# gwenzhang/GGA

Hardware: AMD Instinct MI355X
Metric: kitti_frames_per_sec_gga_train_step (higher is better)
Workload: dtype f32 tensors; products on 2 x f16 operand planes (block-scaled), f32 accumulate - measured no less accurate than fp32 kernels: per convolution 0.7 x (dense) / 0.7-1.2 x (sparse) the RMS error of an fp32 FMA chain vs float64, whole-step losses over 8 seeds <= 2.5e-5 from float64 (fp32 CPU step: <= 1.6

## Files before the change

### gga_amd/csrc/pfn.hip

```cpp
#include "gga_common.h"

__device__ __forceinline__ int64_t pfn_valid_rows(int64_t m, const int32_t* __restrict__ num_valid) {
    if (!num_valid) return m;
    const int64_t v = *num_valid;
    return v < m ? (v < 0 ? 0 : v) : m;
}

#define PFN_C 64
#define PFN_F 10
#define PFN_NM 65
#define PFN_SAVED 238

struct PfnGeom {
    float vx, vy, vz, xo, yo, zo;
};

__device__ __forceinline__ void pfn_decorate(const float4 p, const float mean[3], const float cen[3], float f[PFN_F]) {
    f[0] = p.x - cen[0]; f[1] = p.y - cen[1]; f[2] = p.z - cen[2]; f[3] = p.w;
    f[4] = p.x - mean[0]; f[5] = p.y - mean[1]; f[6] = p.z - mean[2];
    f[7] = f[0]; f[8] = f[1]; f[9] = f[2];
}

__device__ __forceinline__ void pfn_pillar_consts(const float4* __restrict__ pts, int n, const int4 co,
                                                  const PfnGeom g, float mean[3], float cen[3]) {
    float sx = 0.f, sy = 0.f, sz = 0.f;
    for (int p = 0; p < n; ++p) { const float4 q = pts[p]; sx += q.x; sy += q.y; sz += q.z; }
    const float fn = (float)n;
    mean[0] = sx / fn; mean[1] = sy / fn; mean[2] = sz / fn;
    float tx = (float)co.w * g.vx, ty = (float)co.z * g.vy, tz = (float)co.y * g.vz;
    asm volatile("" : "+v"(tx), "+v"(ty), "+v"(tz));
    cen[0] = tx + g.xo; cen[1] = ty + g.yo; cen[2] = tz + g.zo;
}

__global__ __launch_bounds__(256) void pfn_moments_kernel(const float4* __restrict__ voxels,
                                                         const int32_t* __restrict__ num_points,
                                                         const int4* __restrict__ coors, int64_t m,
                                                         const int32_t* __restrict__ num_valid, int P,
                                                         PfnGeom g, double* __restrict__ partials) {
    m = pfn_valid_rows(m, num_valid);
    double acc[PFN_NM];
#pragma unroll
    for (int i = 0; i < PFN_NM; ++i) acc[i] = 0.0;
    for (int64_t v = (int64_t)blockIdx.x * 256 + threadIdx.x; v < m; v += (int64_t)gridDim.x * 256) {
        int n = num_points[v];
        n = n < P ? n : P;
        if (n <= 0) continue;
        const float4* pts = voxels + v * P;
        float mean[3], cen[3];
        pfn_pillar_consts(pts, n, coors[v], g, mean, cen);
        float loc[PFN_NM];
#pragma unroll
        for (int i = 0; i < PFN_NM; ++i) loc[i] = 0.f;
        for (int p = 0; p < n; ++p) {
            float f[PFN_F];
            pfn_decorate(pts[p], mean, cen, f);
            int k = PFN_F;
#pragma unroll
            for (int a = 0; a < PFN_F; ++a) {
                loc[a] += f[a];
#pragma unroll
                for (int b = a; b < PFN_F; ++b) loc[k++] += f[a] * f[b];
            }
        }
#pragma unroll
        for (int i = 0; i < PFN_NM; ++i) acc[i] += (double)loc[i];
    }
    __shared__ double sh[4][PFN_NM];
#pragma unroll
    for (int i = 0; i < PFN_NM; ++i) {
        const double s = wave_sum(acc[i]);
        if ((threadIdx.x & 63) == 0) sh[threadIdx.x >> 6][i] = s;
    }
    __syncthreads();
    if (threadIdx.x < PFN_NM)
        partials[(int64_t)blockIdx.x * PFN_NM + threadIdx.x] =
            (sh[0][threadIdx.x] + sh[1][threadIdx.x]) + (sh[2][threadIdx.x] + sh[3][threadIdx.x]);
}

__global__ __launch_bounds__(64) void pfn_stats_kernel(const double* __restrict__ partials, int nblocks,
                                                      int64_t m, const int32_t* __restrict__ num_valid, int P,
                                                      const float* __restrict__ weight,
                                                      const float* __restrict__ gamma, const float* __restrict__ beta,
                                                      float eps, float momentum, int training,
                                                      float* __restrict__ running_mean, float* __restrict__ running_var,
                                                      double* __restrict__ saved, float* __restrict__ scale_shift) {
    __shared__ double S[PFN_NM];
    const int c = threadIdx.x;
    double rows = (double)pfn_valid_rows(m, num_valid) * (double)P;
    rows = rows > 0.0 ? rows : 1.0;
    if (c == 0) saved[PFN_SAVED] = rows;
    if (training) {
        for (int i = c; i < PFN_NM; i += 64) {
            double s = 0.0;
#pragma unroll 16
            for (int b = 0; b < nblocks; ++b) s += partials[(int64_t)b * PFN_NM + i];
            S[i] = s;
        }
        __syncthreads();
        double S1[PFN_F], S2[PFN_F][PFN_F];
        int k = PFN_F;
        for (int a = 0; a < PFN_F; ++a) {
            S1[a] = S[a];
            for (int b = a; b < PFN_F; ++b) { S2[a][b] = S[k]; S2[b][a] = S[k]; ++k; }
        }
        double w[PFN_F];
        for (int a = 0; a < PFN_F; ++a) w[a] = (double)weight[c * PFN_F + a];
        double m1 = 0.0, m2 = 0.0;
        for (int a = 0; a < PFN_F; ++a) {
            m1 += w[a] * S1[a];
            double t = 0.0;
            for (int b = 0; b < PFN_F; ++b) t += S2[a][b] * w[b];
            m2 += w[a] * t;
        }
        const double mean = m1 / rows;
        double var = m2 / rows - mean * mean;
        var = var > 0.0 ? var : 0.0;
        const double invstd = 1.0 / sqrt(var + (double)eps);
        if (c == 0)
            for (int a = 0; a < PFN_F; ++a) {
                saved[a] = S1[a];
                for (int b = 0; b < PFN_F; ++b) saved[PFN_F + a * PFN_F + b] = S2[a][b];
            }
        saved[110 + c] = mean;
        saved[174 + c] = invstd;
        const float sc = gamma[c] * (float)invstd;
        scale_shift[c] = sc;
        scale_shift[PFN_C + c] = beta[c] - (float)mean * sc;
        const double unb = rows > 1.0 ? var * rows / (rows - 1.0) : var;
        running_mean[c] = (1.0f - momentum) * running_mean[c] + momentum * (float)mean;
        running_var[c] = (1.0f - momentum) * running_var[c] + momentum * (float)unb;
    } else {
        const float invstd = 1.0f / sqrtf(running_var[c] + eps);
        const float sc = gamma[c] * invstd;
        scale_shift[c] = sc;
        scale_shift[PFN_C + c] = beta[c] - running_mean[c] * sc;
    }
}

__global__ __launch_bounds__(256) void pfn_apply_kernel(const float4* __restrict__ voxels,
                                                       const int32_t* __restrict__ num_points,
                                                       const int4* __restrict__ coors, int64_t m,
                                                       const int32_t* __restrict__ num_valid, int P, PfnGeom g,
                                                       const float* __restrict__ weight,
                                                       const float* __restrict__ scale_shift,
                                                       float* __restrict__ out, uint8_t* __restrict__ argmax) {
    const int lane = threadIdx.x & 63;
    const int64_t mv = pfn_valid_rows(m, num_valid);
    float w[PFN_F];
#pragma unroll
    for (int a = 0; a < PFN_F; ++a) w[a] = weight[lane * PFN_F + a];
    const float sc = scale_shift[lane], sh = scale_shift[PFN_C + lane];
    const float ypad = fmaxf(sh, 0.0f);
    const int64_t wave0 = (int64_t)blockIdx.x * 4 + (threadIdx.x >> 6);
    const int64_t nwaves = (int64_t)gridDim.x * 4;
    for (int64_t v = wave0; v < m; v += nwaves) {
        const int64_t vu = __builtin_amdgcn_readfirstlane((int)(v & 0xffffffff)) |
                           ((int64_t)__builtin_amdgcn_readfirstlane((int)(v >> 32)) << 32);
        if (vu >= mv) {
            out[vu * PFN_C + lane] = 0.0f;
            argmax[vu * PFN_C + lane] = 255;
            continue;
        }
        int n = num_points[vu];
        n = n < P ? n : P;
        const float4* pts = voxels + vu * P;
        float best = -INFINITY;
        int bi = 255;
        if (n < P || n <= 0) { best = ypad; }
        if (n > 0) {
            float mean[3], cen[3];
            pfn_pillar_consts(pts, n, coors[vu], g, mean, cen);
            for (int p = 0; p < n; ++p) {
                float f[PFN_F];
                pfn_decorate(pts[p], mean, cen, f);
                float z = 0.0f;
#pragma unroll
                for (int a = 0; a < PFN_F; ++a) z += f[a] * w[a];
                const float y = fmaxf(z * sc + sh, 0.0f);
                if (y > best) { best = y; bi = p; }
            }
        }
        out[vu * PFN_C + lane] = best;
        argmax[vu * PFN_C + lane] = (uint8_t)bi;
    }
}

#define PFN_BW 12

__global__ __launch_bounds__(256) void pfn_bwd_kernel(const float4* __restrict__ voxels,
                                                     const int32_t* __restrict__ num_points,
                                                     const int4* __restrict__ coors, int64_t m,
                                                     const int32_t* __restrict__ num_valid, int P, PfnGeom g,
                                                     const float* __restrict__ weight, const double* __restrict__ saved,
                                                     const float* __restrict__ out, const uint8_t* __restrict__ argmax,
                                                     const float* __restrict__ grad_out, float* __restrict__ partials) {
    const int lane = threadIdx.x & 63;
    float w[PFN_F];
#pragma unroll
    for (int a = 0; a < PFN_F; ++a) w[a] = weight[lane * PFN_F + a];
    const float mean_c = (float)saved[110 + lane], invstd_c = (float)saved[174 + lane];
    float acc[PFN_BW];
#pragma unroll
    for (int i = 0; i < PFN_BW; ++i) acc[i] = 0.0f;
    m = pfn_valid_rows(m, num_valid);
    const int64_t wave0 = (int64_t)blockIdx.x * 4 + (threadIdx.x >> 6);
    const int64_t nwaves = (int64_t)gridDim.x * 4;
    for (int64_t v = wave0; v < m; v += nwaves) {
        const int64_t vu = __builtin_amdgcn_readfirstlane((int)(v & 0xffffffff)) |
                           ((int64_t)__builtin_amdgcn_readfirstlane((int)(v >> 32)) << 32);
        const float y = out[vu * PFN_C + lane];
        const float gy = y > 0.0f ? grad_out[vu * PFN_C + lane] : 0.0f;
        const int bi = argmax[vu * PFN_C + lane];
        int n = num_points[vu];
        n = n < P ? n : P;
        float f[PFN_F];
#pragma unroll
        for (int a = 0; a < PFN_F; ++a) f[a] = 0.0f;
        float z = 0.0f;
        if (n > 0) {
            const float4* pts = voxels + vu * P;
            float mean[3], cen[3];
            pfn_pillar_consts(pts, n, coors[vu], g, mean, cen);
            if (bi != 255) {
                pfn_decorate(pts[bi], mean, cen, f);
#pragma unroll
                for (int a = 0; a < PFN_F; ++a) z += f[a] * w[a];
            }
        }
        const float xhat = (z - mean_c) * invstd_c;
        acc[0] += gy;
        acc[1] += gy * xhat;
#pragma unroll
        for (int a = 0; a < PFN_F; ++a) acc[2 + a] += gy * f[a];
    }
    __shared__ float sh[4][PFN_BW][PFN_C];
#pragma unroll
    for (int i = 0; i < PFN_BW; ++i) sh[threadIdx.x >> 6][i][lane] = acc[i];
    __syncthreads();
    for (int t = threadIdx.x; t < PFN_BW * PFN_C; t += 256) {
        const int i = t / PFN_C, c = t - i * PFN_C;
        partials[(int64_t)blockIdx.x * PFN_BW * PFN_C + t] = (sh[0][i][c] + sh[1][i][c]) + (sh[2][i][c] + sh[3][i][c]);
    }
}

__global__ __launch_bounds__(768) void pfn_bwd_final_kernel(const float* __restrict__ partials, int nblocks,
                                                           const float* __restrict__ weight,
                                                           const float* __restrict__ gamma,
                                                           const double* __restrict__ saved,
                                                           float* __restrict__ grad_weight,
                                                           float* __restrict__ grad_gamma,
                                                           float* __restrict__ grad_beta) {
    __shared__ double red[PFN_BW][PFN_C];
    {
        const int t = threadIdx.x;
        double s = 0.0;
#pragma unroll 16
        for (int b = 0; b < nblocks; ++b) s += (double)partials[(int64_t)b * PFN_BW * PFN_C + t];
        red[t / PFN_C][t % PFN_C] = s;
    }
    __syncthreads();
    if (threadIdx.x >= PFN_C) return;
    const int c = threadIdx.x;
    const double A = red[0][c], Bx = red[1][c];
    const double rows = saved[PFN_SAVED];
    const double mean = saved[110 + c], invstd = saved[174 + c];
    grad_beta[c] = (float)A;
    grad_gamma[c] = (float)Bx;
    const double k = (double)gamma[c] * invstd;
    for (int a = 0; a < PFN_F; ++a) {
        double s2w = 0.0;
        for (int b = 0; b < PFN_F; ++b) s2w += saved[PFN_F + a * PFN_F + b] * (double)weight[c * PFN_F + b];
        const double xf = invstd * (s2w - mean * saved[a]);
        grad_weight[c * PFN_F + a] = (float)(k * (red[2 + a][c] - A / rows * saved[a] - Bx / rows * xf));
    }
}

static int pfn_blocks(int64_t m) {
    int64_t b = (m + 255) / 256;
    return (int)(b < 1 ? 1 : (b > 256 ? 256 : b));
}
static int pfn_wave_blocks(int64_t m) {
    int64_t b = (m + 3) / 4;
    return (int)(b < 1 ? 1 : (b > 512 ? 512 : b));
}

extern "C" size_t gga_pfn_workspace_bytes(int64_t m) {
    const size_t a = (size_t)pfn_blocks(m) * PFN_NM * sizeof(double);
    const size_t b = (size_t)pfn_wave_blocks(m) * PFN_BW * PFN_C * sizeof(float);
    return gga_align_up(a > b ? a : b, 256) + 2 * PFN_C * sizeof(float);
}

static int pfn_check(const char* fn, const gga_pfn_params* prm, int64_t m, int P) {
    GGA_REQUIRE(prm, "%s: null params", fn);
    GGA_REQUIRE(m >= 1 && P >= 1 && P <= 254, "%s: bad sizes (m=%lld, max_points=%d; need 1..254)", fn, (long long)m, P);
    GGA_REQUIRE(prm->channels == PFN_C && prm->in_features == 4,
                "%s: the fused kernel is specialised for 4 point features -> %d channels (got %d -> %d)", fn, PFN_C,
                prm->in_features, prm->channels);
    return GGA_OK;
}

extern "C" int gga_pfn_fwd(const float* voxels, const int32_t* num_points, const int32_t* coors, int64_t m,
                           const int32_t* num_valid, int P, const gga_pfn_params* prm, const float* weight, const float* gamma, const float* beta,
                           float* running_mean, float* running_var, float* out, uint8_t* argmax, double* saved,
                           void* workspace, size_t workspace_bytes, void* stream_) {
    hipStream_t stream = (hipStream_t)stream_;
    if (int rc = pfn_check("gga_pfn_fwd", prm, m, P)) return rc;
    GGA_REQUIRE(voxels && num_points && coors && weight && gamma && beta && running_mean && running_var && out &&
                    argmax && saved && workspace,
                "gga_pfn_fwd: null pointer argument");
    if (workspace_bytes < gga_pfn_workspace_bytes(m)) {
        gga_set_error("gga_pfn_fwd: workspace %zu B < required %zu B", workspace_bytes, gga_pfn_workspace_bytes(m));
        return GGA_ERR_WORKSPACE;
    }
    const PfnGeom g = { prm->voxel_size[0], prm->voxel_size[1], prm->voxel_size[2],
                        prm->offsets[0], prm->offsets[1], prm->offsets[2] };
    double* partials = (double*)workspace;
    float* scale_shift = (float*)((char*)workspace + gga_pfn_workspace_bytes(m) - 2 * PFN_C * sizeof(float));
    const int nb = pfn_blocks(m);
    if (prm->training) {
        hipLaunchKernelGGL(pfn_moments_kernel, dim3(nb), dim3(256), 0, stream, (const float4*)voxels, num_points,
                           (const int4*)coors, m, num_valid, P, g, partials);
        GGA_CHECK_LAUNCH("pfn_moments_kernel");
    }
    hipLaunchKernelGGL(pfn_stats_kernel, dim3(1), dim3(64), 0, stream, partials, nb, m, num_valid, P, weight,
                       gamma, beta, prm->eps, prm->momentum, prm->training, running_mean, running_var, saved,
                       scale_shift);
    GGA_CHECK_LAUNCH("pfn_stats_kernel");
    hipLaunchKernelGGL(pfn_apply_kernel, dim3(pfn_wave_blocks(m)), dim3(256), 0, stream, (const float4*)voxels,
                       num_points, (const int4*)coors, m, num_valid, P, g, weight, scale_shift, out, argmax);
    GGA_CHECK_LAUNCH("pfn_apply_kernel");
    return GGA_OK;
}

extern "C" int gga_pfn_bwd(const float* voxels, const int32_t* num_points, const int32_t* coors, int64_t m,
                           const int32_t* num_valid, int P, const gga_pfn_params* prm, const float* weight, const float* gamma, const float* out,
                           const uint8_t* argmax, const double* saved, const float* grad_out, float* grad_weight,
                           float* grad_gamma, float* grad_beta, void* workspace, size_t workspace_bytes,
                           void* stream_) {
    hipStream_t stream = (hipStream_t)stream_;
    if (int rc = pfn_check("gga_pfn_bwd", prm, m, P)) return rc;
    GGA_REQUIRE(voxels && num_points && coors && weight && gamma && out && argmax && saved && grad_out &&
                    grad_weight && grad_gamma && grad_beta && workspace,
                "gga_pfn_bwd: null pointer argument");
    GGA_REQUIRE(prm->training, "gga_pfn_bwd: backward is defined for training-mode batch statistics");
    if (workspace_bytes < gga_pfn_workspace_bytes(m)) {
        gga_set_error("gga_pfn_bwd: workspace %zu B < required %zu B", workspace_bytes, gga_pfn_workspace_bytes(m));
        return GGA_ERR_WORKSPACE;
    }
    const PfnGeom g = { prm->voxel_size[0], prm->voxel_size[1], prm->voxel_size[2],
                        prm->offsets[0], prm->offsets[1], prm->offsets[2] };
    const int nb = pfn_wave_blocks(m);
    hipLaunchKernelGGL(pfn_bwd_kernel, dim3(nb), dim3(256), 0, stream, (const float4*)voxels, num_points,
                       (const int4*)coors, m, num_valid, P, g, weight, saved, out, argmax, grad_out, (float*)workspace);
    GGA_CHECK_LAUNCH("pfn_bwd_kernel");
    hipLaunchKernelGGL(pfn_bwd_final_kernel, dim3(1), dim3(PFN_BW * PFN_C), 0, stream, (const float*)workspace, nb,
                       weight, gamma, saved, grad_weight, grad_gamma, grad_beta);
    GGA_CHECK_LAUNCH("pfn_bwd_final_kernel");
    return GGA_OK;
}
```

### gga_amd/csrc/weight_bank.hip

```cpp
#include "gga_common.h"
#include "conv_planes.h"

struct PackEntry {
    const float* src;
    uint16_t* dst;
    const uint32_t* amax;
    int64_t s_k0, s_k1, s_c, s_col;
    int64_t first;
    int32_t kw, kvol, n_c, n_col, c0, col0, n_in, co, layout, reverse;
};
static_assert(sizeof(PackEntry) == sizeof(GgaPackEntry), "PackEntry must match the ABI struct");

struct AmaxEntry {
    const float* src;
    uint32_t* slot;
    int64_t n;
    int64_t first_block;
};
static_assert(sizeof(AmaxEntry) == sizeof(GgaAmaxEntry), "AmaxEntry must match the ABI struct");

template <typename E, typename F>
__device__ __forceinline__ int find_entry(const E* __restrict__ t, int n, int64_t i, F first_of) {
    int lo = 0, hi = n - 1;
    while (lo < hi) {
        const int mid = (lo + hi + 1) >> 1;
        if (first_of(t[mid]) <= i) lo = mid; else hi = mid - 1;
    }
    return lo;
}

#define WB_AMAX_PER_BLOCK (256 * 8)

__global__ __launch_bounds__(256) void wb_absmax_kernel(const AmaxEntry* __restrict__ table, int n_entries) {
    const int e = find_entry(table, n_entries, (int64_t)blockIdx.x, [](const AmaxEntry& a) { return a.first_block; });
    const AmaxEntry en = table[e];
    const int64_t base = ((int64_t)blockIdx.x - en.first_block) * WB_AMAX_PER_BLOCK;
    uint32_t m = 0;
#pragma unroll
    for (int u = 0; u < 8; ++u) {
        const int64_t i = base + u * 256 + threadIdx.x;
        if (i < en.n) {
            const uint32_t q = __float_as_uint(en.src[i]) & 0x7FFFFFFFu;
            if (q < 0x7F800000u && q > m) m = q;
        }
    }
#pragma unroll
    for (int o = 32; o > 0; o >>= 1) { const uint32_t t = __shfl_xor(m, o, 64); m = t > m ? t : m; }
    __shared__ uint32_t wm[4];
    if ((threadIdx.x & 63) == 0) wm[threadIdx.x >> 6] = m;
    __syncthreads();
    if (threadIdx.x == 0) {
        m = max(max(wm[0], wm[1]), max(wm[2], wm[3]));
        if (m > __hip_atomic_load(en.slot, __ATOMIC_RELAXED, __HIP_MEMORY_SCOPE_AGENT)) atomicMax(en.slot, m);
    }
}

__global__ __launch_bounds__(256) void wb_pack_kernel(const PackEntry* __restrict__ table, int n_entries, int64_t total, int np) {
    const int64_t i = (int64_t)blockIdx.x * 256 + threadIdx.x;
    if (i >= total) return;
    const int e = find_entry(table, n_entries, i, [](const PackEntry& a) { return a.first; });
    const PackEntry en = table[e];
    int64_t j = i - en.first;
    const int cl = (int)(j % en.n_c); j /= en.n_c;
    const int colloc = (int)(j % en.n_col);
    const int tap = (int)(j / en.n_col);
    const int t = en.reverse ? en.kvol - 1 - tap : tap;
    const int k0 = t / en.kw, k1 = t - k0 * en.kw;
    const float v = en.src[k0 * en.s_k0 + k1 * en.s_k1 + cl * en.s_c + colloc * en.s_col];
    const int c = en.c0 + cl, col = en.col0 + colloc;
    const int nchunks = (en.n_in + MF_TK - 1) / MF_TK;
    uint16_t* dst;
    int64_t plane;
    if (en.layout == 0) {
        const int ch = c & 31;
        const int64_t stage = (int64_t)tap * nchunks + (c >> 5);
        plane = (int64_t)en.co * 32;
        dst = en.dst + stage * (np * plane) + (int64_t)col * 32 + ((((ch >> 3) ^ ((col >> 2) & 3)) << 3) | (ch & 7));
    } else {
        const int64_t stage16 = (int64_t)tap * (2 * nchunks) + (c >> 4);
        plane = (int64_t)en.co * 16;
        dst = en.dst + stage16 * (np * plane) + (int64_t)col * 16 + (c & 15);
    }
    if (np == 3) {
        uint32_t p1, p2, p3;
        x9_split(v, p1, p2, p3);
        dst[0] = (uint16_t)p1; dst[plane] = (uint16_t)p2; dst[2 * plane] = (uint16_t)p3;
    } else {
        uint32_t w0, w1;
        h2_split2(v * h2_scale(h2_scale_exp(*en.amax)), 0.0f, w0, w1);
        dst[0] = (uint16_t)(w0 & 0xFFFFu); dst[plane] = (uint16_t)(w1 & 0xFFFFu);
    }
}

extern "C" int64_t gga_absmax_table_blocks(int64_t n) { return n <= 0 ? 0 : (n + WB_AMAX_PER_BLOCK - 1) / WB_AMAX_PER_BLOCK; }

extern "C" int gga_absmax_table(const GgaAmaxEntry* table_device, int n_entries, int64_t n_blocks, uint32_t* slots,
                                int n_slots, void* stream_) {
    hipStream_t stream = (hipStream_t)stream_;
    GGA_REQUIRE(table_device && slots && n_entries >= 0 && n_slots >= 0 && n_blocks >= 0 && n_blocks < 2147483647ll,
                "gga_absmax_table: bad arguments");
    if (n_slots) GGA_CHECK_HIP(hipMemsetAsync(slots, 0, (size_t)n_slots * sizeof(uint32_t), stream), "gga_absmax_table: memset");
    if (n_entries == 0 || n_blocks == 0) return GGA_OK;
    hipLaunchKernelGGL(wb_absmax_kernel, dim3((unsigned)n_blocks), dim3(256), 0, stream, (const AmaxEntry*)table_device, n_entries);
    GGA_CHECK_LAUNCH("wb_absmax_kernel");
    return GGA_OK;
}

extern "C" int gga_pack_weights_table(const GgaPackEntry* table_device, int n_entries, int64_t total, int planes, void* stream_) {
    hipStream_t stream = (hipStream_t)stream_;
    GGA_REQUIRE(table_device && n_entries >= 0 && total >= 0 && (planes == 2 || planes == 3), "gga_pack_weights_table: bad arguments");
    if (n_entries == 0 || total == 0) return GGA_OK;
    const int64_t nb = (total + 255) / 256;
    GGA_REQUIRE(nb < 2147483647ll, "gga_pack_weights_table: too many elements for one launch");
    hipLaunchKernelGGL(wb_pack_kernel, dim3((unsigned)nb), dim3(256), 0, stream, (const PackEntry*)table_device, n_entries, total, planes);
    GGA_CHECK_LAUNCH("wb_pack_kernel");
    return GGA_OK;
}
```

Measured before the change: 548.3.

## Add pipelined PFN apply/backward kernels and vectorized weight-bank packing

Adds new PFN forward-apply and backward kernels in which each lane loads one pillar's header, first points and mean/center, then broadcasts them across the wave with readlane. The backward kernel batches out/grad/argmax loads 16 at a time. The stats and final-reduction kernels are templated on unroll factor, with 64 used on the new path. The weight-bank pack gets a fast kernel that looks up the table entry once per wave via ballot and writes 8 packed elements per thread with 16-byte stores. Both new paths are on by default behind env toggles, at the cost of more complex index math, extra registers, and a fallback path for unaligned pieces.

```diff
diff --git a/gga_amd/csrc/pfn.hip b/gga_amd/csrc/pfn.hip
--- a/gga_amd/csrc/pfn.hip
+++ b/gga_amd/csrc/pfn.hip
@@ -77,6 +77,54 @@
             (sh[0][threadIdx.x] + sh[1][threadIdx.x]) + (sh[2][threadIdx.x] + sh[3][threadIdx.x]);
 }
 
+struct PfnLaneHead { int n; int4 co; };
+
+__device__ __forceinline__ int pfn_clamp_n(int n, int P) {
+    n = n < P ? n : P;
+    return n > 0 ? n : 0;
+}
+
+__device__ __forceinline__ float pfn_lane(float v, int l) {
+    return __int_as_float(__builtin_amdgcn_readlane(__float_as_int(v), l));
+}
+
+__device__ __forceinline__ PfnLaneHead pfn_lane_head(const int32_t* __restrict__ num_points, const int4* __restrict__ coors,
+                                                     int64_t v, int P) {
+    PfnLaneHead h;
+    h.n = pfn_clamp_n(num_points[v], P);
+    h.co = coors[v];
+    return h;
+}
+
+__device__ __forceinline__ void pfn_lane_points(const float4* __restrict__ pts, int n, float4 q[4]) {
+    const int last = n > 0 ? n - 1 : 0;
+#pragma unroll
+    for (int i = 0; i < 4; ++i) q[i] = pts[i < last ? i : last];
+}
+
+__device__ __forceinline__ void pfn_lane_consts(const float4* __restrict__ pts, const PfnLaneHead h, const float4 q[4],
+                                                const PfnGeom g, float mean[3], float cen[3]) {
+    const int n = h.n, last = n > 0 ? n - 1 : 0;
+    float sx = 0.f, sy = 0.f, sz = 0.f;
+#pragma unroll
+    for (int i = 0; i < 4; ++i)
+        if (i < n) { sx += q[i].x; sy += q[i].y; sz += q[i].z; }
+    for (int p0 = 4; p0 < n; p0 += 4) {
+        float4 t[4];
+#pragma unroll
+        for (int i = 0; i < 4; ++i) t[i] = pts[p0 + i < last ? p0 + i : last];
+#pragma unroll
+        for (int i = 0; i < 4; ++i)
+            if (p0 + i < n) { sx += t[i].x; sy += t[i].y; sz += t[i].z; }
+    }
+    const float fn = (float)n;
+    mean[0] = sx / fn; mean[1] = sy / fn; mean[2] = sz / fn;
+    float tx = (float)h.co.w * g.vx, ty = (float)h.co.z * g.vy, tz = (float)h.co.y * g.vz;
+    asm volatile("" : "+v"(tx), "+v"(ty), "+v"(tz));
+    cen[0] = tx + g.xo; cen[1] = ty + g.yo; cen[2] = tz + g.zo;
+}
+
+template <int U>
 __global__ __launch_bounds__(64) void pfn_stats_kernel(const double* __restrict__ partials, int nblocks,
                                                       int64_t m, const int32_t* __restrict__ num_valid, int P,
                                                       const float* __restrict__ weight,
@@ -92,7 +140,7 @@
     if (training) {
         for (int i = c; i < PFN_NM; i += 64) {
             double s = 0.0;
-#pragma unroll 16
+#pragma unroll U
             for (int b = 0; b < nblocks; ++b) s += partials[(int64_t)b * PFN_NM + i];
             S[i] = s;
         }
@@ -243,6 +291,149 @@
     }
 }
 
+__global__ __launch_bounds__(256) void pfn_apply_pipe_kernel(const float4* __restrict__ voxels,
+                                                            const int32_t* __restrict__ num_points,
+                                                            const int4* __restrict__ coors, int64_t m,
+                                                            const int32_t* __restrict__ num_valid, int P, PfnGeom g,
+                                                            const float* __restrict__ weight,
+                                                            const float* __restrict__ scale_shift,
+                                                            float* __restrict__ out, uint8_t* __restrict__ argmax) {
+    const int lane = threadIdx.x & 63;
+    const int64_t mv = pfn_valid_rows(m, num_valid);
+    const int64_t v0 = ((int64_t)blockIdx.x * 4 + __builtin_amdgcn_readfirstlane((int)(threadIdx.x >> 6))) * 64;
+    if (v0 >= m) return;
+    float w[PFN_F];
+#pragma unroll
+    for (int a = 0; a < PFN_F; ++a) w[a] = weight[lane * PFN_F + a];
+    const float sc = scale_shift[lane], sh = scale_shift[PFN_C + lane];
+    const float ypad = fmaxf(sh, 0.0f);
+    const int64_t vl = v0 + lane < mv ? v0 + lane : (mv > 0 ? mv - 1 : 0);
+    const PfnLaneHead h = pfn_lane_head(num_points, coors, vl, P);
+    float4 q[4];
+    float lmean[3], lcen[3];
+    pfn_lane_points(voxels + vl * P, h.n, q);
+    pfn_lane_consts(voxels + vl * P, h, q, g, lmean, lcen);
+    const int cnt = (int)(m - v0 < 64 ? m - v0 : 64);
+    for (int j = 0; j < cnt; ++j) {
+        const int64_t v = v0 + j;
+        if (v >= mv) {
+            out[v * PFN_C + lane] = 0.0f;
+            argmax[v * PFN_C + lane] = 255;
+            continue;
+        }
+        const int n = __builtin_amdgcn_readlane(h.n, j);
+        float best = -INFINITY;
+        int bi = 255;
+        if (n < P || n <= 0) { best = ypad; }
+        if (n > 0) {
+            float mean[3], cen[3];
+#pragma unroll
+            for (int i = 0; i < 3; ++i) { mean[i] = pfn_lane(lmean[i], j); cen[i] = pfn_lane(lcen[i], j); }
+            auto point = [&](const float4 pt, int p) {
+                float f[PFN_F];
+                pfn_decorate(pt, mean, cen, f);
+                float z = 0.0f;
+#pragma unroll
+                for (int a = 0; a < PFN_F; ++a) z += f[a] * w[a];
+                const float y = fmaxf(z * sc + sh, 0.0f);
+                if (y > best) { best = y; bi = p; }
+            };
+#pragma unroll
+            for (int i = 0; i < 4; ++i)
+                if (i < n) point(make_float4(pfn_lane(q[i].x, j), pfn_lane(q[i].y, j), pfn_lane(q[i].z, j), pfn_lane(q[i].w, j)), i);
+            const float4* pts = voxels + v * P;
+            for (int p = 4; p < n; ++p) point(pts[p], p);
+        }
+        out[v * PFN_C + lane] = best;
+        argmax[v * PFN_C + lane] = (uint8_t)bi;
+    }
+}
+
+template <int DB>
+__global__ __launch_bounds__(256) void pfn_bwd_pipe_kernel(const float4* __restrict__ voxels,
+                                                          const int32_t* __restrict__ num_points,
+                                                          const int4* __restrict__ coors, int64_t m,
+                                                          const int32_t* __restrict__ num_valid, int P, PfnGeom g,
+                                                          const float* __restrict__ weight, const double* __restrict__ saved,
+                                                          const float* __restrict__ out, const uint8_t* __restrict__ argmax,
+                                                          const float* __restrict__ grad_out, float* __restrict__ partials) {
+    const int lane = threadIdx.x & 63;
+    float w[PFN_F];
+#pragma unroll
+    for (int a = 0; a < PFN_F; ++a) w[a] = weight[lane * PFN_F + a];
+    const float mean_c = (float)saved[110 + lane], invstd_c = (float)saved[174 + lane];
+    float acc[PFN_BW];
+#pragma unroll
+    for (int i = 0; i < PFN_BW; ++i) acc[i] = 0.0f;
+    m = pfn_valid_rows(m, num_valid);
+    const int64_t wave0 = (int64_t)blockIdx.x * 4 + __builtin_amdgcn_readfirstlane((int)(threadIdx.x >> 6));
+    const int64_t nwaves = (int64_t)gridDim.x * 4;
+    const int K = wave0 < m ? (int)((m - wave0 + nwaves - 1) / nwaves) : 0;
+    for (int kc = 0; kc < K; kc += 64) {
+        const int64_t vl = wave0 + (int64_t)(kc + lane < K ? kc + lane : K - 1) * nwaves;
+        const PfnLaneHead h = pfn_lane_head(num_points, coors, vl, P);
+        float lmean[3], lcen[3];
+        {
+            float4 q[4];
+            pfn_lane_points(voxels + vl * P, h.n, q);
+            pfn_lane_consts(voxels + vl * P, h, q, g, lmean, lcen);
+        }
+        const int cnt = K - kc < 64 ? K - kc : 64;
+        for (int jb = 0; jb < cnt; jb += DB) {
+            float y[DB], go[DB];
+            int bi[DB];
+            float4 ap[DB];
+#pragma unroll
+            for (int d = 0; d < DB; ++d) {
+                const int64_t v = wave0 + (int64_t)(jb + d < cnt ? kc + jb + d : K - 1) * nwaves;
+                y[d] = out[v * PFN_C + lane];
+                go[d] = grad_out[v * PFN_C + lane];
+                bi[d] = argmax[v * PFN_C + lane];
+            }
+#pragma unroll
+            for (int d = 0; d < DB; ++d) {
+                const int64_t v = wave0 + (int64_t)(jb + d < cnt ? kc + jb + d : K - 1) * nwaves;
+                ap[d] = voxels[v * P + (bi[d] < P ? bi[d] : 0)];
+            }
+#pragma unroll
+            for (int d = 0; d < DB; ++d) {
+                const int j = jb + d;
+                if (j >= cnt) continue;
+                const float gy = y[d] > 0.0f ? go[d] : 0.0f;
+                const int n = __builtin_amdgcn_readlane(h.n, j);
+                float f[PFN_F];
+#pragma unroll
+                for (int i = 0; i < PFN_F; ++i) f[i] = 0.0f;
+                float z = 0.0f;
+                if (n > 0) {
+                    float mean[3], cen[3];
+#pragma unroll
+                    for (int i = 0; i < 3; ++i) { mean[i] = pfn_lane(lmean[i], j); cen[i] = pfn_lane(lcen[i], j); }
+                    if (bi[d] != 255) {
+                        pfn_decorate(ap[d], mean, cen, f);
+#pragma unroll
+                        for (int i = 0; i < PFN_F; ++i) z += f[i] * w[i];
+                    }
+                }
+                const float xhat = (z - mean_c) * invstd_c;
+                acc[0] += gy;
+                acc[1] += gy * xhat;
+#pragma unroll
+                for (int i = 0; i < PFN_F; ++i) acc[2 + i] += gy * f[i];
+            }
+        }
+    }
+    __shared__ float sh[4][PFN_BW][PFN_C];
+#pragma unroll
+    for (int i = 0; i < PFN_BW; ++i) sh[threadIdx.x >> 6][i][lane] = acc[i];
+    __syncthreads();
+    for (int t = threadIdx.x; t < PFN_BW * PFN_C; t += 256) {
+        const int i = t / PFN_C, c = t - i * PFN_C;
+        partials[(int64_t)blockIdx.x * PFN_BW * PFN_C + t] = (sh[0][i][c] + sh[1][i][c]) + (sh[2][i][c] + sh[3][i][c]);
+    }
+}
+
+template <int U>
 __global__ __launch_bounds__(768) void pfn_bwd_final_kernel(const float* __restrict__ partials, int nblocks,
                                                            const float* __restrict__ weight,
                                                            const float* __restrict__ gamma,
@@ -254,7 +445,7 @@
     {
         const int t = threadIdx.x;
         double s = 0.0;
-#pragma unroll 16
+#pragma unroll U
         for (int b = 0; b < nblocks; ++b) s += (double)partials[(int64_t)b * PFN_BW * PFN_C + t];
         red[t / PFN_C][t % PFN_C] = s;
     }
@@ -283,6 +474,12 @@
     int64_t b = (m + 3) / 4;
     return (int)(b < 1 ? 1 : (b > 512 ? 512 : b));
 }
+static int64_t pfn_apply_pipe_blocks(int64_t m) { return (m + 255) / 256; }
+static bool pfn_pipelined() {
+    const char* e = getenv("GGA_PFN_PIPELINED");
+    return !(e && atoi(e) == 0);
+}
+#define PFN_BWD_BATCH 16
 
 extern "C" size_t gga_pfn_workspace_bytes(int64_t m) {
     const size_t a = (size_t)pfn_blocks(m) * PFN_NM * sizeof(double);
@@ -317,17 +514,28 @@
     double* partials = (double*)workspace;
     float* scale_shift = (float*)((char*)workspace + gga_pfn_workspace_bytes(m) - 2 * PFN_C * sizeof(float));
     const int nb = pfn_blocks(m);
+    const bool pipe = pfn_pipelined();
     if (prm->training) {
         hipLaunchKernelGGL(pfn_moments_kernel, dim3(nb), dim3(256), 0, stream, (const float4*)voxels, num_points,
                            (const int4*)coors, m, num_valid, P, g, partials);
         GGA_CHECK_LAUNCH("pfn_moments_kernel");
     }
-    hipLaunchKernelGGL(pfn_stats_kernel, dim3(1), dim3(64), 0, stream, partials, nb, m, num_valid, P, weight,
-                       gamma, beta, prm->eps, prm->momentum, prm->training, running_mean, running_var, saved,
-                       scale_shift);
+    if (pipe)
+        hipLaunchKernelGGL(pfn_stats_kernel<64>, dim3(1), dim3(64), 0, stream, partials, nb, m, num_valid, P, weight,
+                           gamma, beta, prm->eps, prm->momentum, prm->training, running_mean, running_var, saved,
+                           scale_shift);
+    else
+        hipLaunchKernelGGL(pfn_stats_kernel<16>, dim3(1), dim3(64), 0, stream, partials, nb, m, num_valid, P, weight,
+                           gamma, beta, prm->eps, prm->momentum, prm->training, running_mean, running_var, saved,
+                           scale_shift);
     GGA_CHECK_LAUNCH("pfn_stats_kernel");
-    hipLaunchKernelGGL(pfn_apply_kernel, dim3(pfn_wave_blocks(m)), dim3(256), 0, stream, (const float4*)voxels,
-                       num_points, (const int4*)coors, m, num_valid, P, g, weight, scale_shift, out, argmax);
+    if (pipe)
+        hipLaunchKernelGGL(pfn_apply_pipe_kernel, dim3((unsigned)pfn_apply_pipe_blocks(m)), dim3(256), 0, stream,
+                           (const float4*)voxels, num_points, (const int4*)coors, m, num_valid, P, g, weight, scale_shift, out,
+                           argmax);
+    else
+        hipLaunchKernelGGL(pfn_apply_kernel, dim3(pfn_wave_blocks(m)), dim3(256), 0, stream, (const float4*)voxels,
+                           num_points, (const int4*)coors, m, num_valid, P, g, weight, scale_shift, out, argmax);
     GGA_CHECK_LAUNCH("pfn_apply_kernel");
     return GGA_OK;
 }
@@ -350,11 +558,20 @@
     const PfnGeom g = { prm->voxel_size[0], prm->voxel_size[1], prm->voxel_size[2],
                         prm->offsets[0], prm->offsets[1], prm->offsets[2] };
     const int nb = pfn_wave_blocks(m);
-    hipLaunchKernelGGL(pfn_bwd_kernel, dim3(nb), dim3(256), 0, stream, (const float4*)voxels, num_points,
-                       (const int4*)coors, m, num_valid, P, g, weight, saved, out, argmax, grad_out, (float*)workspace);
+    const bool pipe = pfn_pipelined();
+    if (pipe)
+        hipLaunchKernelGGL(pfn_bwd_pipe_kernel<PFN_BWD_BATCH>, dim3(nb), dim3(256), 0, stream, (const float4*)voxels, num_points,
+                           (const int4*)coors, m, num_valid, P, g, weight, saved, out, argmax, grad_out, (float*)workspace);
+    else
+        hipLaunchKernelGGL(pfn_bwd_kernel, dim3(nb), dim3(256), 0, stream, (const float4*)voxels, num_points,
+                           (const int4*)coors, m, num_valid, P, g, weight, saved, out, argmax, grad_out, (float*)workspace);
     GGA_CHECK_LAUNCH("pfn_bwd_kernel");
-    hipLaunchKernelGGL(pfn_bwd_final_kernel, dim3(1), dim3(PFN_BW * PFN_C), 0, stream, (const float*)workspace, nb,
-                       weight, gamma, saved, grad_weight, grad_gamma, grad_beta);
+    if (pipe)
+        hipLaunchKernelGGL(pfn_bwd_final_kernel<64>, dim3(1), dim3(PFN_BW * PFN_C), 0, stream, (const float*)workspace, nb,
+                           weight, gamma, saved, grad_weight, grad_gamma, grad_beta);
+    else
+        hipLaunchKernelGGL(pfn_bwd_final_kernel<16>, dim3(1), dim3(PFN_BW * PFN_C), 0, stream, (const float*)workspace, nb,
+                           weight, gamma, saved, grad_weight, grad_gamma, grad_beta);
     GGA_CHECK_LAUNCH("pfn_bwd_final_kernel");
     return GGA_OK;
 }
diff --git a/gga_amd/csrc/weight_bank.hip b/gga_amd/csrc/weight_bank.hip
--- a/gga_amd/csrc/weight_bank.hip
+++ b/gga_amd/csrc/weight_bank.hip
@@ -55,12 +55,7 @@
     }
 }
 
-__global__ __launch_bounds__(256) void wb_pack_kernel(const PackEntry* __restrict__ table, int n_entries, int64_t total, int np) {
-    const int64_t i = (int64_t)blockIdx.x * 256 + threadIdx.x;
-    if (i >= total) return;
-    const int e = find_entry(table, n_entries, i, [](const PackEntry& a) { return a.first; });
-    const PackEntry en = table[e];
-    int64_t j = i - en.first;
+__device__ __forceinline__ void wb_pack_element(const PackEntry& en, int64_t j, int np) {
     const int cl = (int)(j % en.n_c); j /= en.n_c;
     const int colloc = (int)(j % en.n_col);
     const int tap = (int)(j / en.n_col);
@@ -92,6 +87,115 @@
     }
 }
 
+__global__ __launch_bounds__(256) void wb_pack_kernel(const PackEntry* __restrict__ table, int n_entries, int64_t total, int np) {
+    const int64_t i = (int64_t)blockIdx.x * 256 + threadIdx.x;
+    if (i >= total) return;
+    const int e = find_entry(table, n_entries, i, [](const PackEntry& a) { return a.first; });
+    const PackEntry en = table[e];
+    wb_pack_element(en, i - en.first, np);
+}
+
+template <typename E, typename F>
+__device__ __forceinline__ int find_entry_wave(const E* __restrict__ t, int n, int64_t i, F first_of) {
+    const int lane = threadIdx.x & 63;
+    int cnt = 0;
+    for (int b = 0; b < n; b += 256) {
+        bool le[4];
+#pragma unroll
+        for (int u = 0; u < 4; ++u) {
+            const int k = b + u * 64 + lane;
+            le[u] = k < n && first_of(t[k < n ? k : n - 1]) <= i;
+        }
+#pragma unroll
+        for (int u = 0; u < 4; ++u) cnt += __popcll(__ballot(le[u]));
+    }
+    return cnt > 0 ? cnt - 1 : 0;
+}
+
+#define WB_PIECE 8
+
+__global__ __launch_bounds__(256) void wb_pack_fast_kernel(const PackEntry* __restrict__ table, int n_entries, int64_t total, int np) {
+    const int64_t iw = ((int64_t)blockIdx.x * 256 + __builtin_amdgcn_readfirstlane((int)(threadIdx.x & ~63u))) * WB_PIECE;
+    if (iw >= total) return;
+    const int64_t i0 = iw + (int64_t)(threadIdx.x & 63) * WB_PIECE;
+    if (i0 >= total) return;
+    int e = find_entry_wave(table, n_entries, iw, [](const PackEntry& a) { return a.first; });
+    while (e + 1 < n_entries && table[e + 1].first <= i0) ++e;
+    const PackEntry en = table[e];
+    const int64_t next = e + 1 < n_entries ? table[e + 1].first : total;
+    const int64_t j = i0 - en.first;
+    const int64_t per_tap = (int64_t)en.n_c * en.n_col;
+    const bool whole = i0 + WB_PIECE <= next && i0 + WB_PIECE <= total && ((en.n_c | en.c0 | (int)j) & (WB_PIECE - 1)) == 0 &&
+                       ((uintptr_t)en.dst & 15) == 0 && per_tap * en.kvol < (int64_t)1 << 31 && en.kvol > 0;
+    if (!whole) {
+        for (int u = 0; u < WB_PIECE && i0 + u < total; ++u) {
+            const int64_t i = i0 + u;
+            int eu = e;
+            while (eu + 1 < n_entries && table[eu + 1].first <= i) ++eu;
+            const PackEntry eni = table[eu];
+            wb_pack_element(eni, i - eni.first, np);
+        }
+        return;
+    }
+    const int64_t st_tap = en.kw > 1 ? en.s_k1 : en.s_k0, st_col = en.s_col, st_c = en.s_c;
+    const int rank_tap = (st_col < st_tap) + (st_c < st_tap), rank_col = (st_tap <= st_col) + (st_c < st_col),
+              rank_c = (st_tap <= st_c) + (st_col <= st_c);
+    const uint32_t nc8 = (uint32_t)en.n_c / WB_PIECE;
+    const uint32_t e0 = rank_tap == 0 ? (uint32_t)en.kvol : (rank_col == 0 ? (uint32_t)en.n_col : nc8);
+    const uint32_t e1 = rank_tap == 1 ? (uint32_t)en.kvol : (rank_col == 1 ? (uint32_t)en.n_col : nc8);
+    const uint32_t jp = (uint32_t)j / WB_PIECE, r = jp / e0, x0 = jp - r * e0, x2 = r / e1, x1 = r - x2 * e1;
+    const int tap = (int)(rank_tap == 0 ? x0 : (rank_tap == 1 ? x1 : x2));
+    const int colloc = (int)(rank_col == 0 ? x0 : (rank_col == 1 ? x1 : x2));
+    const int cl = (int)(rank_c == 0 ? x0 : (rank_c == 1 ? x1 : x2)) * WB_PIECE;
+    const int t = en.reverse ? en.kvol - 1 - tap : tap;
+    const int k0 = t / en.kw, k1 = t - k0 * en.kw;
+    const float* __restrict__ src = en.src + (k0 * en.s_k0 + k1 * en.s_k1 + cl * en.s_c + colloc * en.s_col);
+    float v[WB_PIECE];
+#pragma unroll
+    for (int u = 0; u < WB_PIECE; ++u) v[u] = src[u * en.s_c];
+    const int c = en.c0 + cl, col = en.col0 + colloc;
+    const int nchunks = (en.n_in + MF_TK - 1) / MF_TK;
+    uint16_t* dst;
+    int64_t plane;
+    if (en.layout == 0) {
+        const int ch = c & 31;
+        const int64_t stage = (int64_t)tap * nchunks + (c >> 5);
+        plane = (int64_t)en.co * 32;
+        dst = en.dst + stage * (np * plane) + (int64_t)col * 32 + ((((ch >> 3) ^ ((col >> 2) & 3)) << 3) | (ch & 7));
+    } else {
+        const int64_t stage16 = (int64_t)tap * (2 * nchunks) + (c >> 4);
+        plane = (int64_t)en.co * 16;
+        dst = en.dst + stage16 * (np * plane) + (int64_t)col * 16 + (c & 15);
+    }
+    uint32_t w1[WB_PIECE / 2], w2[WB_PIECE / 2], w3[WB_PIECE / 2];
+    if (np == 3) {
+#pragma unroll
+        for (int u = 0; u < WB_PIECE; u += 2) {
+            uint32_t a1, a2, a3, b1, b2, b3;
+            x9_split(v[u], a1, a2, a3);
+            x9_split(v[u + 1], b1, b2, b3);
+            w1[u / 2] = (a1 & 0xFFFFu) | (b1 << 16); w2[u / 2] = (a2 & 0xFFFFu) | (b2 << 16); w3[u / 2] = (a3 & 0xFFFFu) | (b3 << 16);
+        }
+        *(uint4*)(dst + 2 * plane) = make_uint4(w3[0], w3[1], w3[2], w3[3]);
+    } else {
+        const float scale = h2_scale(h2_scale_exp(*en.amax));
+#pragma unroll
+        for (int u = 0; u < WB_PIECE; u += 2) {
+            uint32_t a0, a1, b0, b1;
+            h2_split2(v[u] * scale, 0.0f, a0, a1);
+            h2_split2(v[u + 1] * scale, 0.0f, b0, b1);
+            w1[u / 2] = (a0 & 0xFFFFu) | (b0 << 16); w2[u / 2] = (a1 & 0xFFFFu) | (b1 << 16);
+        }
+    }
+    *(uint4*)dst = make_uint4(w1[0], w1[1], w1[2], w1[3]);
+    *(uint4*)(dst + plane) = make_uint4(w2[0], w2[1], w2[2], w2[3]);
+}
+
+static bool wb_fast() {
+    const char* e = getenv("GGA_WB_FAST");
+    return !(e && atoi(e) == 0);
+}
+
 extern "C" int64_t gga_absmax_table_blocks(int64_t n) { return n <= 0 ? 0 : (n + WB_AMAX_PER_BLOCK - 1) / WB_AMAX_PER_BLOCK; }
 
 extern "C" int gga_absmax_table(const GgaAmaxEntry* table_device, int n_entries, int64_t n_blocks, uint32_t* slots,
@@ -112,7 +216,11 @@
     if (n_entries == 0 || total == 0) return GGA_OK;
     const int64_t nb = (total + 255) / 256;
     GGA_REQUIRE(nb < 2147483647ll, "gga_pack_weights_table: too many elements for one launch");
-    hipLaunchKernelGGL(wb_pack_kernel, dim3((unsigned)nb), dim3(256), 0, stream, (const PackEntry*)table_device, n_entries, total, planes);
+    if (wb_fast())
+        hipLaunchKernelGGL(wb_pack_fast_kernel, dim3((unsigned)((nb + WB_PIECE - 1) / WB_PIECE)), dim3(256), 0, stream,
+                           (const PackEntry*)table_device, n_entries, total, planes);
+    else
+        hipLaunchKernelGGL(wb_pack_kernel, dim3((unsigned)nb), dim3(256), 0, stream, (const PackEntry*)table_device, n_entries, total, planes);
     GGA_CHECK_LAUNCH("wb_pack_kernel");
     return GGA_OK;
 }
```

Measured after the change: 547.1. Within noise of the previous version (-0.2%).
